# slackhq/nebula

Measured on AMD Instinct MI355X. Metric: GiB/s device-resident AES-256-GCM seal+open, 1300 B pkts, 64 Ki batch, higher is better.
Workload: dtype u8; 1 GPU; C2 AES-256-GCM, 1 tunnel key, 65536 x 1300 B packets, device-resident; packets_per_gpu=65536, payload_bytes_per_pkt=1300, keys=1, cipher=AES-256-GCM, parallelism=1 GPU(s), independent packet shards, no collective

## Files before the change

### nebula_amd/csrc/aes_gcm.hip

```cpp
#include <hip/hip_runtime.h>

#include <atomic>
#include <hip/hip_ext.h>

#include <cstdlib>
#include <cstring>
#include <stdint.h>

#include <type_traits>

#include "../../include/nebula_aead.h"
#include "device_common.hpp"
#include "knobs.hpp"
#include "layout.hpp"
#include "rxwin.hpp"
#include "sched.hpp"
#include "timing.hpp"

#ifdef NEB_ISA_MARKS
#define NEB_MARK(x) asm volatile(";NEBMARK " #x)
#else
#define NEB_MARK(x) ((void)0)
#endif

namespace neb {


struct T0Table {
    uint32_t t[256];
};
constexpr uint8_t kSbox[256] = {
    0x63,0x7c,0x77,0x7b,0xf2,0x6b,0x6f,0xc5,0x30,0x01,0x67,0x2b,0xfe,0xd7,0xab,0x76,
    0xca,0x82,0xc9,0x7d,0xfa,0x59,0x47,0xf0,0xad,0xd4,0xa2,0xaf,0x9c,0xa4,0x72,0xc0,
    0xb7,0xfd,0x93,0x26,0x36,0x3f,0xf7,0xcc,0x34,0xa5,0xe5,0xf1,0x71,0xd8,0x31,0x15,
    0x04,0xc7,0x23,0xc3,0x18,0x96,0x05,0x9a,0x07,0x12,0x80,0xe2,0xeb,0x27,0xb2,0x75,
    0x09,0x83,0x2c,0x1a,0x1b,0x6e,0x5a,0xa0,0x52,0x3b,0xd6,0xb3,0x29,0xe3,0x2f,0x84,
    0x53,0xd1,0x00,0xed,0x20,0xfc,0xb1,0x5b,0x6a,0xcb,0xbe,0x39,0x4a,0x4c,0x58,0xcf,
    0xd0,0xef,0xaa,0xfb,0x43,0x4d,0x33,0x85,0x45,0xf9,0x02,0x7f,0x50,0x3c,0x9f,0xa8,
    0x51,0xa3,0x40,0x8f,0x92,0x9d,0x38,0xf5,0xbc,0xb6,0xda,0x21,0x10,0xff,0xf3,0xd2,
    0xcd,0x0c,0x13,0xec,0x5f,0x97,0x44,0x17,0xc4,0xa7,0x7e,0x3d,0x64,0x5d,0x19,0x73,
    0x60,0x81,0x4f,0xdc,0x22,0x2a,0x90,0x88,0x46,0xee,0xb8,0x14,0xde,0x5e,0x0b,0xdb,
    0xe0,0x32,0x3a,0x0a,0x49,0x06,0x24,0x5c,0xc2,0xd3,0xac,0x62,0x91,0x95,0xe4,0x79,
    0xe7,0xc8,0x37,0x6d,0x8d,0xd5,0x4e,0xa9,0x6c,0x56,0xf4,0xea,0x65,0x7a,0xae,0x08,
    0xba,0x78,0x25,0x2e,0x1c,0xa6,0xb4,0xc6,0xe8,0xdd,0x74,0x1f,0x4b,0xbd,0x8b,0x8a,
    0x70,0x3e,0xb5,0x66,0x48,0x03,0xf6,0x0e,0x61,0x35,0x57,0xb9,0x86,0xc1,0x1d,0x9e,
    0xe1,0xf8,0x98,0x11,0x69,0xd9,0x8e,0x94,0x9b,0x1e,0x87,0xe9,0xce,0x55,0x28,0xdf,
    0x8c,0xa1,0x89,0x0d,0xbf,0xe6,0x42,0x68,0x41,0x99,0x2d,0x0f,0xb0,0x54,0xbb,0x16};

constexpr uint8_t xt(uint8_t a) { return (uint8_t)((a << 1) ^ ((a & 0x80) ? 0x1b : 0)); }
constexpr T0Table make_t0() {
    T0Table r{};
    for (int i = 0; i < 256; i++) {
        uint32_t s = kSbox[i], s2 = xt(kSbox[i]), s3 = s2 ^ s;
        r.t[i] = s2 | (s << 8) | (s << 16) | (s3 << 24);
    }
    return r;
}
__constant__ T0Table c_T0 = make_t0();


__device__ __forceinline__ uint32_t x3(uint32_t a, uint32_t b, uint32_t c) {
    uint32_t r;
    asm("v_bitop3_b32 %0, %1, %2, %3 bitop3:0x96" : "=v"(r) : "v"(a), "v"(b), "v"(c));
    return r;
}
__device__ __forceinline__ uint32_t x3s(uint32_t a, uint32_t b, uint32_t k) {
    uint32_t r;
    asm("v_bitop3_b32 %0, %1, %2, %3 bitop3:0x96" : "=v"(r) : "v"(a), "v"(b), "s"(k));
    return r;
}
__device__ __forceinline__ uint32_t rotl8(uint32_t x) { return __builtin_amdgcn_alignbit(x, x, 24); }
__device__ __forceinline__ uint4 xor4(uint4 a, uint4 b) { return make_uint4(a.x ^ b.x, a.y ^ b.y, a.z ^ b.z, a.w ^ b.w); }
__device__ __forceinline__ uint4 x34(uint4 a, uint4 b, uint4 c) {
    return make_uint4(x3(a.x, b.x, c.x), x3(a.y, b.y, c.y), x3(a.z, b.z, c.z), x3(a.w, b.w, c.w));
}
__device__ __forceinline__ uint4 sel4(bool c, uint4 a, uint4 b) {
    return make_uint4(c ? a.x : b.x, c ? a.y : b.y, c ? a.z : b.z, c ? a.w : b.w);
}
__device__ __forceinline__ uint4 bswap4(uint4 v) { return make_uint4(bswap32(v.x), bswap32(v.y), bswap32(v.z), bswap32(v.w)); }
__device__ __forceinline__ uint4 shfl_xor4(uint4 v, int m) {
    return make_uint4(__shfl_xor(v.x, m), __shfl_xor(v.y, m), __shfl_xor(v.z, m), __shfl_xor(v.w, m));
}
__device__ __forceinline__ uint32_t byte_of(uint32_t w, int k) {
    return k == 0 ? (w & 0xFFu) : (k == 3 ? (w >> 24) : __builtin_amdgcn_ubfe(w, 8 * k, 8));
}

template <class T>
__device__ __forceinline__ T lds_at(const void* base, uint32_t byte_off) {
    return *reinterpret_cast<const T*>(
        __builtin_assume_aligned(reinterpret_cast<const char*>(base) + byte_off, sizeof(T)));
}

__device__ __forceinline__ uint2 lds_b64(const void* base, uint32_t byte_off) {
    typedef uint32_t v2u __attribute__((ext_vector_type(2)));
    typedef const volatile __attribute__((address_space(3))) v2u* lds_ptr;
    const v2u v = *(lds_ptr)__builtin_assume_aligned(reinterpret_cast<const char*>(base) + byte_off, 8);
    return make_uint2(v.x, v.y);
}

__device__ __forceinline__ uint2 ttab_lane_base(uint32_t lane, uint32_t high = 0u) {
    const uint32_t c = lane & 31u, hi = c >> 4;
    return make_uint2((c << 3) | (hi << 2) | high, (c << 3) | ((hi ^ 1u) << 2) | high);
}
__device__ __forceinline__ uint2 ttab_entry(uint32_t i) {
    const uint32_t t = c_T0.t[i >> 5], t2 = __builtin_amdgcn_alignbit(t, t, 16);
    return (i & 16u) ? make_uint2(t2, t) : make_uint2(t, t2);
}

#ifndef NEB_PRIO
#define NEB_PRIO 3
#endif
#ifndef NEB_PRIO_AGE
#define NEB_PRIO_AGE 1
#endif

struct RkRegs {
    const uint32_t* k;
    static constexpr bool kUniform = true;
    static constexpr int kPrioHi = NEB_PRIO, kPrioLo = 0;
    __device__ __forceinline__ uint4 get(int r) const {
        return make_uint4(k[4 * r], k[4 * r + 1], k[4 * r + 2], k[4 * r + 3]);
    }
};
template <int HI, int LO>
struct RkRegsPrio : RkRegs {
    static constexpr int kPrioHi = HI, kPrioLo = LO;
};
struct RkLds {
    const uint4* base;
    static constexpr bool kUniform = false;
    static constexpr int kPrioHi = NEB_PRIO, kPrioLo = 0;
    __device__ __forceinline__ uint4 get(int r) const { return base[r]; }
};

struct TLook {
    const uint2* ttab;
    uint2 lb;
    __device__ __forceinline__ uint32_t t0(uint32_t s, int k) const {
        return lds_at<uint32_t>(ttab, perm(s, lb.x, 0x0C020000u | ((4u + (uint32_t)k) << 8)));
    }
    __device__ __forceinline__ uint32_t t2(uint32_t s, int k) const {
        return lds_at<uint32_t>(ttab, perm(s, lb.y, 0x0C020000u | ((4u + (uint32_t)k) << 8)));
    }
    __device__ __forceinline__ uint32_t t1(uint32_t s, int k) const { return rotl8(t0(s, k)); }
    __device__ __forceinline__ uint32_t t3(uint32_t s, int k) const { return rotl8(t2(s, k)); }
    __device__ __forceinline__ uint32_t t1r(uint32_t s, int k) const { return t0(s, k); }
    __device__ __forceinline__ uint32_t t3r(uint32_t s, int k) const { return t2(s, k); }
    static constexpr bool kFour = false;
};

__device__ __forceinline__ uint32_t ttab4_lane_base(uint32_t lane) {
    const uint32_t c = lane & 31u, hi = c >> 4;
    return ((c << 3) | (hi << 2)) | (1u << 16) | (((c << 3) | ((hi ^ 1u) << 2)) << 24);
}
__device__ __forceinline__ uint2 ttab4_entry(uint32_t i) {
    uint32_t t = c_T0.t[(i >> 5) & 255u];
    if (i & 8192u) t = __builtin_amdgcn_alignbit(t, t, 16);
    const uint32_t t1 = rotl8(t);
    return (i & 16u) ? make_uint2(t1, t) : make_uint2(t, t1);
}
template <uint32_t N, uint32_t THREADS, class F>
__device__ __forceinline__ void fill_ttab(uint2* dst, uint32_t tid, F entry) {
    constexpr uint32_t K = (N + THREADS - 1) / THREADS;
    constexpr bool kWhole = N % THREADS == 0;
    uint2 v[K];
#pragma unroll
    for (uint32_t j = 0; j < K; j++) v[j] = entry((tid + j * THREADS) % N);
#pragma unroll
    for (uint32_t j = 0; j < K; j++)
        if (kWhole || tid + j * THREADS < N) dst[tid + j * THREADS] = v[j];
}
struct TLook4 {
    const uint2* ttab;
    uint32_t lb;
    __device__ __forceinline__ uint32_t at(uint32_t s, int k, uint32_t sel) const {
        return lds_at<uint32_t>(ttab, perm(s, lb, sel | ((4u + (uint32_t)k) << 8)));
    }
    __device__ __forceinline__ uint32_t t0(uint32_t s, int k) const { return at(s, k, 0x0C0C0000u); }
    __device__ __forceinline__ uint32_t t1(uint32_t s, int k) const { return at(s, k, 0x0C0C0003u); }
    __device__ __forceinline__ uint32_t t2(uint32_t s, int k) const { return at(s, k, 0x0C020000u); }
    __device__ __forceinline__ uint32_t t3(uint32_t s, int k) const { return at(s, k, 0x0C020003u); }
    __device__ __forceinline__ uint32_t t1r(uint32_t s, int k) const { return t1(s, k); }
    __device__ __forceinline__ uint32_t t3r(uint32_t s, int k) const { return t3(s, k); }
    static constexpr bool kFour = true;
};

template <int FIRST, class TL, class RK>
__device__ __forceinline__ uint4 aes256_rounds(uint32_t s0, uint32_t s1, uint32_t s2, uint32_t s3, const TL& T,
                                               const RK& rk) {
    uint4 k;
#pragma unroll
    for (int r = FIRST; r < 14; r++) {
        k = rk.get(r);
#if NEB_PRIO
        __builtin_amdgcn_sched_barrier(0);
        __builtin_amdgcn_s_setprio(RK::kPrioHi);
#endif
        const uint32_t a0 = T.t0(s0, 0), a1 = T.t1r(s1, 1), a2 = T.t2(s2, 2), a3 = T.t3r(s3, 3);
        const uint32_t b0 = T.t0(s1, 0), b1 = T.t1r(s2, 1), b2 = T.t2(s3, 2), b3 = T.t3r(s0, 3);
        const uint32_t c0 = T.t0(s2, 0), c1 = T.t1r(s3, 1), c2 = T.t2(s0, 2), c3 = T.t3r(s1, 3);
        const uint32_t d0 = T.t0(s3, 0), d1 = T.t1r(s0, 1), d2 = T.t2(s1, 2), d3 = T.t3r(s2, 3);
#if NEB_PRIO
        __builtin_amdgcn_sched_barrier(0);
        __builtin_amdgcn_s_setprio(RK::kPrioLo);
#endif
        if constexpr (TL::kFour) {
            if constexpr (RK::kUniform) {
                s0 = x3s(x3(a0, a1, a2), a3, k.x);
                s1 = x3s(x3(b0, b1, b2), b3, k.y);
                s2 = x3s(x3(c0, c1, c2), c3, k.z);
                s3 = x3s(x3(d0, d1, d2), d3, k.w);
            } else {
                s0 = x3(x3(a0, a1, a2), a3, k.x);
                s1 = x3(x3(b0, b1, b2), b3, k.y);
                s2 = x3(x3(c0, c1, c2), c3, k.z);
                s3 = x3(x3(d0, d1, d2), d3, k.w);
            }
        } else if constexpr (RK::kUniform) {
            s0 = x3s(a0, a2, k.x) ^ rotl8(a1 ^ a3);
            s1 = x3s(b0, b2, k.y) ^ rotl8(b1 ^ b3);
            s2 = x3s(c0, c2, k.z) ^ rotl8(c1 ^ c3);
            s3 = x3s(d0, d2, k.w) ^ rotl8(d1 ^ d3);
        } else {
            s0 = x3(a0, a2, k.x) ^ rotl8(a1 ^ a3);
            s1 = x3(b0, b2, k.y) ^ rotl8(b1 ^ b3);
            s2 = x3(c0, c2, k.z) ^ rotl8(c1 ^ c3);
            s3 = x3(d0, d2, k.w) ^ rotl8(d1 ^ d3);
        }
    }
    k = rk.get(14);
#if NEB_PRIO
    __builtin_amdgcn_sched_barrier(0);
    __builtin_amdgcn_s_setprio(RK::kPrioHi);
#endif
    const uint32_t a0 = T.t0(s0, 0), a1 = T.t0(s1, 1), a2 = T.t0(s2, 2), a3 = T.t0(s3, 3);
    const uint32_t b0 = T.t0(s1, 0), b1 = T.t0(s2, 1), b2 = T.t0(s3, 2), b3 = T.t0(s0, 3);
    const uint32_t c0 = T.t0(s2, 0), c1 = T.t0(s3, 1), c2 = T.t0(s0, 2), c3 = T.t0(s1, 3);
    const uint32_t d0 = T.t0(s3, 0), d1 = T.t0(s0, 1), d2 = T.t0(s1, 2), d3 = T.t0(s2, 3);
#if NEB_PRIO
    __builtin_amdgcn_sched_barrier(0);
    __builtin_amdgcn_s_setprio(RK::kPrioLo);
#endif
    uint4 o;
    if constexpr (RK::kUniform) {
        o.x = x3s(perm(a1, a0, 0x0C0C0501u), perm(a3, a2, 0x05010C0Cu), k.x);
        o.y = x3s(perm(b1, b0, 0x0C0C0501u), perm(b3, b2, 0x05010C0Cu), k.y);
        o.z = x3s(perm(c1, c0, 0x0C0C0501u), perm(c3, c2, 0x05010C0Cu), k.z);
        o.w = x3s(perm(d1, d0, 0x0C0C0501u), perm(d3, d2, 0x05010C0Cu), k.w);
    } else {
        o.x = x3(perm(a1, a0, 0x0C0C0501u), perm(a3, a2, 0x05010C0Cu), k.x);
        o.y = x3(perm(b1, b0, 0x0C0C0501u), perm(b3, b2, 0x05010C0Cu), k.y);
        o.z = x3(perm(c1, c0, 0x0C0C0501u), perm(c3, c2, 0x05010C0Cu), k.z);
        o.w = x3(perm(d1, d0, 0x0C0C0501u), perm(d3, d2, 0x05010C0Cu), k.w);
    }
    return o;
}

template <class TL, class RK>
__device__ __forceinline__ uint4 aes256_block(uint32_t s0, uint32_t s1, uint32_t s2, uint32_t s3, const TL& T,
                                              const RK& rk) {
    const uint4 k = rk.get(0);
    return aes256_rounds<1>(s0 ^ k.x, s1 ^ k.y, s2 ^ k.z, s3 ^ k.w, T, rk);
}

struct CtrConst {
    uint4 K, L;
    uint32_t k0w;
};

template <class TL, class RK>
__device__ __forceinline__ CtrConst aes_ctr_prep(uint32_t c1, uint32_t c2, const TL& T, const RK& rk) {
    const uint4 k0 = rk.get(0), k1 = rk.get(1), k2 = rk.get(2);
    const uint32_t s0 = k0.x, s1 = c1 ^ k0.y, s2 = c2 ^ k0.z, s3 = k0.w;
    CtrConst c;
    c.k0w = k0.w;
    c.K.x = T.t0(s0, 0) ^ rotl8(T.t0(s1, 1)) ^ T.t2(s2, 2) ^ k1.x;
    c.K.y = T.t0(s1, 0) ^ rotl8(T.t0(s2, 1)) ^ rotl8(T.t2(s0, 3)) ^ k1.y;
    c.K.z = T.t0(s2, 0) ^ rotl8(T.t0(s3, 1) ^ T.t2(s1, 3)) ^ T.t2(s0, 2) ^ k1.z;
    c.K.w = T.t0(s3, 0) ^ rotl8(T.t0(s0, 1) ^ T.t2(s2, 3)) ^ T.t2(s1, 2) ^ k1.w;
    c.L.x = T.t2(c.K.z, 2) ^ rotl8(T.t2(c.K.w, 3)) ^ k2.x;
    c.L.y = rotl8(T.t0(c.K.z, 1)) ^ T.t2(c.K.w, 2) ^ k2.y;
    c.L.z = T.t0(c.K.z, 0) ^ rotl8(T.t0(c.K.w, 1)) ^ k2.z;
    c.L.w = T.t0(c.K.w, 0) ^ rotl8(T.t2(c.K.z, 3)) ^ k2.w;
    return c;
}

template <class TL, class RK>
__device__ __forceinline__ uint4 aes256_ctr_block(const CtrConst& c, uint32_t ctr, const TL& T, const RK& rk) {
    const uint32_t s3 = c.k0w ^ bswap32(ctr);
    const uint32_t t0 = c.K.x ^ T.t3(s3, 3);
    const uint32_t t1 = c.K.y ^ T.t2(s3, 2);
    const uint32_t u0 = x3(c.L.x, T.t0(t0, 0), T.t1(t1, 1));
    const uint32_t u1 = x3(c.L.y, T.t0(t1, 0), T.t3(t0, 3));
    const uint32_t u2 = x3(c.L.z, T.t2(t0, 2), T.t3(t1, 3));
    const uint32_t u3 = x3(c.L.w, T.t2(t1, 2), T.t1(t0, 1));
    return aes256_rounds<3>(u0, u1, u2, u3, T, rk);
}

template <class TL, class RK>
__device__ __forceinline__ CtrConst aes_ctr_prep8(uint32_t c1, uint32_t c2, const TL& T, const RK& rk) {
    CtrConst c = aes_ctr_prep(c1, c2, T, rk);
    const uint4 k2 = rk.get(2);
    c.K.y ^= T.t2(c.k0w, 2);
    c.L.x = rotl8(T.t0(c.K.y, 1)) ^ T.t2(c.K.z, 2) ^ rotl8(T.t2(c.K.w, 3)) ^ k2.x;
    c.L.y = T.t0(c.K.y, 0) ^ rotl8(T.t0(c.K.z, 1)) ^ T.t2(c.K.w, 2) ^ k2.y;
    c.L.z = T.t0(c.K.z, 0) ^ rotl8(T.t0(c.K.w, 1) ^ T.t2(c.K.y, 3)) ^ k2.z;
    c.L.w = T.t0(c.K.w, 0) ^ T.t2(c.K.y, 2) ^ rotl8(T.t2(c.K.z, 3)) ^ k2.w;
    return c;
}

template <class TL, class RK>
__device__ __forceinline__ uint4 aes256_ctr8_block(const CtrConst& c, uint32_t ctr, const TL& T, const RK& rk) {
    const uint32_t t0 = c.K.x ^ T.t3(c.k0w ^ (ctr << 24), 3);
    const uint32_t u0 = c.L.x ^ T.t0(t0, 0);
    const uint32_t u1 = c.L.y ^ T.t3(t0, 3);
    const uint32_t u2 = c.L.z ^ T.t2(t0, 2);
    const uint32_t u3 = c.L.w ^ T.t1(t0, 1);
    return aes256_rounds<3>(u0, u1, u2, u3, T, rk);
}


__device__ __forceinline__ uint4 gf_mulx(uint4 v) {
    uint32_t lsb = v.w & 1u;
// ... 567 lines not shown
        constexpr int CM = decltype(cm)::value;
        CtrConst cc{};
        if constexpr (CM == 2) cc = aes_ctr_prep8(c1, c2, T, rk);
        else if constexpr (CM == 1) cc = aes_ctr_prep(c1, c2, T, rk);
        NEB_MARK(ctr_done);
        auto fast_round = [&](const LaneBlock& b) {
            const uint32_t off = 16u * (b.k - 1u);
            return __all(b.is_ct && off + 16u <= d.len && off >= hdr &&
                         ((d.dst_off | (uint32_t)(uintptr_t)args.arena) & 15u) == 0u);
        };
        auto fast_load = [&](const LaneBlock& b) {
            const uint8_t* sp = args.arena + d.src_off + 16u * (b.k - 1u);
            return __all(((uint32_t)(uintptr_t)sp & 3u) == 0u) ? load_u4_a4(sp) : load_shifted16(sp);
        };
        auto io = [&](const LaneBlock& b, uint4 G, uint4 ks, bool fast, uint4 pre) {
            const uint32_t off = 16u * (b.k - 1u);
            if (fast) {
                const uint4 in = pre;
                if constexpr (CS) {
                    if (cs_on) cs_acc += le16_sum(in);
                }
                const uint4 out = xor4(in, ks);
                *reinterpret_cast<uint4*>(args.arena + d.dst_off + off) = out;
                A = xor4(G, bswap4(OPEN ? in : out));
                return;
            }
            const uint4 in = gcm_lane_load(d, b, args.arena, hdr);
            if constexpr (CS) {
                if (cs_on && b.is_ct) {
                    const uint32_t off = 16u * (b.k - 1u);
                    const uint32_t hi = min(16u, d.len - off), lo = hdr > off ? min(hdr - off, 16u) : 0u;
                    if (lo < hi) {
                        const uint4 v = mask_block(in, hi);
                        cs_acc += le16_sum(xor4(v, mask_block(v, lo)));
                    }
                    if (cs_f - off < 16u) {
                        const uint32_t q = cs_f - off;
                        cs_fk = (block_byte(in, q) << 24) | (block_byte(in, q + 1u) << 16) | (block_byte(ks, q) << 8) |
                                block_byte(ks, q + 1u);
                    }
                }
            }
            A = xor4(G, gcm_lane_io<OPEN>(d, b, in, ks, args.arena, ej0));
        };
        auto horner = [&](uint32_t r) -> uint4 { return r == 0 ? make_uint4(0, 0, 0, 0) : gh.horner(A, lg); };
        auto tround = [&](uint32_t r) {
            NEB_MARK(round_begin);
            if (r < sh.R) {
                const LaneBlock b = lane_block(sh, r, l, lg);
                const bool fast = fast_round(b);
                uint4 pre = make_uint4(0, 0, 0, 0);
                if (fast) pre = fast_load(b);
                const uint4 G = horner(r);
                __builtin_amdgcn_sched_barrier(0);
                uint4 ks = make_uint4(0, 0, 0, 0);
                if (__any(b.is_ct || b.is_len)) ks = gcm_lane_ks<CM>(b, c1, c2, cc, T, rk);
                io(b, G, ks, fast, pre);
            }
            NEB_MARK(round_end);
        };
        for (uint32_t r = 0; __any(r < sh.R); r++) tround(r);
    };
#if NEB_ONE_TRACE
    const uint64_t tp0 = __builtin_amdgcn_s_memrealtime();
#endif
    if (__all(sh.m + 1u < 256u)) rounds(std::integral_constant<int, 2>{});
    else if (__all(sh.m + 1u < 65536u)) rounds(std::integral_constant<int, 1>{});
    else rounds(std::integral_constant<int, 0>{});
    if constexpr (CS) {
        for (uint32_t sft = 1; sft < LPP; sft <<= 1) {
            cs_acc += (uint32_t)__shfl_xor((int)cs_acc, (int)sft);
            cs_fk |= (uint32_t)__shfl_xor((int)cs_fk, (int)sft);
        }
    }
#if NEB_ONE_TRACE
    __builtin_amdgcn_s_waitcnt(0);
    const uint64_t tp1 = __builtin_amdgcn_s_memrealtime();
#endif
#ifdef NEB_WAVE_TRACE
    const uint64_t tq2 = phase_now();
    phase_add(1, tq1, tq2);
#endif
    NEB_MARK(rounds_done);
    uint4 V = gh.final(A, lane, lg);
    NEB_MARK(final_done);
#ifdef NEB_WAVE_TRACE
    const uint64_t tq3 = phase_now();
    phase_add(2, tq2, tq3);
#endif
#if NEB_ONE_TRACE
    __builtin_amdgcn_s_waitcnt(0);
    const uint64_t tp2 = __builtin_amdgcn_s_memrealtime();
    if (lane == 0) printf("  rounds %u  final %u (x10 ns, R=%u)\n", (unsigned)(tp1 - tp0), (unsigned)(tp2 - tp1), sh.R);
#endif
    if constexpr (CS) {
        if (run && cs_on && l == LPP - 1u) V = xor4(V, gcm_csum_fix(d, sh.n, sh.na, cs_acc, cs_fk, args.arena, cs_pow));
    }
    if (run && gcm_finish<OPEN>(d, V, ej0.get(), lane, l, LPP, args.arena)) st = NEB_STATUS_AUTH_FAILED;
    if (valid && l == LPP - 1u) args.status[p] = (int32_t)st;
    NEB_MARK(grp_end);
#ifdef NEB_WAVE_TRACE
    phase_add(3, tq3, phase_now());
#endif
}

__device__ __forceinline__ void load_round_keys(const uint32_t* rec, uint32_t rks[60]) {
#pragma unroll
    for (int i = 0; i < 60; i++) rks[i] = __builtin_amdgcn_readfirstlane(rec[kRecRoundKeys + i]);
}

#ifdef NEB_WAVE_TRACE
constexpr uint32_t kWaveTraceSlots = 64, kWaveTraceWaves = 8192, kWaveTraceCap = kWaveTraceSlots * kWaveTraceWaves;
__device__ uint4 g_wtrace[kWaveTraceCap];
__device__ __forceinline__ void wave_trace(uint32_t lane, uint32_t slot, uint32_t a, uint32_t b, uint64_t t0,
                                           uint64_t t1) {
    const uint32_t w = blockIdx.x * (blockDim.x >> 6) + (threadIdx.x >> 6);
    if (lane == 0u && w < kWaveTraceWaves && slot < kWaveTraceSlots)
        g_wtrace[w * kWaveTraceSlots + slot] = make_uint4(a | 0x80000000u, b, (uint32_t)t0, (uint32_t)t1);
}
#endif


constexpr int kSingleWaves = 16;
constexpr int kSingleWpe = 4;
constexpr int kSingleThreads = kSingleWaves * kWave;

struct SingleLds {
#if NEB_GHASH5
    uint2 full[2 * kWin5 * 32];
#else
    uint4 full[32 * 16];
#endif
    uint4 pos1[8 * 16];
    uint2 ttab[2 * 256 * 32];
    uint4 pos23[2][8 * 16];
#if NEB_GHASH5
    uint4 pos4[8 * 16];
#endif
};
struct SingleLdsCs : SingleLds {
    uint4 pow2[10 * 16];
};

template <bool OPEN, bool CS = false, bool RX = false>
__global__ __launch_bounds__(kSingleThreads, kSingleWpe) void gcm_single_kernel(GcmArgs args) {
    __shared__ std::conditional_t<CS, SingleLdsCs, SingleLds> lds;
    const uint32_t tid = threadIdx.x;
    const uint32_t lane = tid & 63u;
    const uint32_t wave = tid >> 6;
    const uint32_t* srec = args.keys + (size_t)args.key_hint * kKeyRecDwords;
#ifdef NEB_WAVE_TRACE
    const uint64_t tk0 = __builtin_amdgcn_s_memrealtime();
#endif
    uint4 r_full = make_uint4(0, 0, 0, 0), r_h = make_uint4(0, 0, 0, 0), r_p = make_uint4(0, 0, 0, 0);
#if NEB_GHASH5
    static_assert(kSingleThreads >= kWin5 * 32, "one window-table entry per thread");
    const uint32_t f5_p = tid >> 5, f5_v = tid & 31u;
    if (tid < (uint32_t)kWin5 * 32u) {
#pragma unroll
        for (uint32_t j = 0; j < 5u; j++) {
            const uint32_t b = 5u * f5_p + j, bc = min(b, 127u);
            const uint4 c = ld_rec4(srec, kRecFull + 4u * ((bc >> 2) * 16u + (8u >> (bc & 3u))));
            const uint32_t m = (b < 128u && ((f5_v >> (4u - j)) & 1u)) ? ~0u : 0u;
            r_full = make_uint4(r_full.x ^ (c.x & m), r_full.y ^ (c.y & m), r_full.z ^ (c.z & m), r_full.w ^ (c.w & m));
        }
    }
    if (tid < 128u) r_h = ld_rec4(srec, kRecPos1 + 4u * tid);
    if (tid < 384u) r_p = ld_rec4(srec, (tid < 128u ? kRecPos2 : tid < 256u ? kRecPos3 : kRecFull) + 4u * (tid & 127u));
#else
    static_assert(kSingleThreads >= 512, "one full-table entry per thread");
    if (tid < 512u) r_full = ld_rec4(srec, kRecFull + 4u * tid);
    if (tid < 128u) r_h = ld_rec4(srec, kRecPos1 + 4u * tid);
    if (tid < 256u) r_p = ld_rec4(srec, (tid < 128u ? kRecPos2 : kRecPos3) + 4u * (tid & 127u));
#endif
    const TLook4 T{lds.ttab, ttab4_lane_base(lane)};
    fill_ttab<2u * 256u * 32u, kSingleThreads>(lds.ttab, tid, ttab4_entry);
#if NEB_GHASH5
    if (tid < (uint32_t)kWin5 * 32u) {
        lds.full[(2u * f5_p) * 32u + f5_v] = make_uint2(r_full.x, r_full.y);
        lds.full[(2u * f5_p + 1u) * 32u + f5_v] = make_uint2(r_full.z, r_full.w);
    }
    if (tid >= 256u && tid < 384u) lds.pos4[tid & 127u] = r_p;
#else
    if (tid < 512u) lds.full[tid] = r_full;
#endif
    if (tid < 128u) lds.pos1[tid] = r_h;
    if (tid < 256u) lds.pos23[tid >> 7][tid & 127u] = r_p;

    const uint4* cs_pow = nullptr;
    if constexpr (CS) {
        if (tid < 160u) lds.pow2[tid] = ld_rec4(srec, rec_shoup_pow2(tid >> 4) + 4u * (tid & 15u));
        cs_pow = lds.pow2;
    }
    uint32_t rks[60];
    load_round_keys(srec, rks);
    __syncthreads();
    const RkRegs rk{rks};
#if NEB_GHASH5
    const uint32_t tab_off[4] = {(uint32_t)offsetof(SingleLds, pos4), (uint32_t)offsetof(SingleLds, pos23[1]),
#else
    const uint32_t tab_off[4] = {(uint32_t)offsetof(SingleLds, full), (uint32_t)offsetof(SingleLds, pos23[1]),
#endif
                                 (uint32_t)offsetof(SingleLds, pos23[0]), (uint32_t)offsetof(SingleLds, pos1)};
    const GhFullPerm gh{lds.full, &lds, final_perm_lanes(lane, tab_off)};

    const bool key_ok = __builtin_amdgcn_readfirstlane(srec[kRecAlg]) == NEB_ALG_AESGCM;
    uint32_t npkt = args.npkt;
    if (args.npkt_dev) npkt = min(npkt, __builtin_amdgcn_readfirstlane(*args.npkt_dev));
    const uint32_t ngroups = (npkt + kPpw - 1u) / kPpw;
    const uint32_t slots = gridDim.x * kSingleWaves;
    uint32_t main_groups = ngroups;
    if (args.tail_slots && ngroups > slots && ngroups % slots)
        main_groups = ngroups / slots * slots;
#ifdef NEB_WAVE_TRACE
    uint32_t trace_k = 1;
    wave_trace(lane, 0, blockIdx.x << 20 | wave << 16, ~0u, tk0, __builtin_amdgcn_s_memrealtime());
#endif
    auto groups = [&](const auto& rkp) {
        for (uint32_t grp = blockIdx.x + wave * gridDim.x; grp < main_groups; grp += slots) {
#ifdef NEB_WAVE_TRACE
            const uint64_t tc0 = __builtin_amdgcn_s_memrealtime();
#endif
            const uint32_t p = grp * kPpw + lane / kLpp;
            gcm_packet_group<OPEN, CS, RX>(args, p, p < npkt, args.key_hint, key_ok, rkp, gh, T, lane, kLg, cs_pow);
#ifdef NEB_WAVE_TRACE
            wave_trace(lane, trace_k++, blockIdx.x << 20 | wave << 16 | 16u << 8 | 2u << 4 | 1u, grp, tc0,
                       __builtin_amdgcn_s_memrealtime());
#endif
        }
    };
#if NEB_PRIO && NEB_PRIO_AGE
    if (__builtin_amdgcn_readfirstlane(wave) >> 3) groups(RkRegsPrio<NEB_PRIO, 1>{rk});
    else groups(rk);
#else
    groups(rk);
#endif
}

constexpr uint32_t kTailLg = 6, kTailPpw = kWave >> kTailLg;
constexpr uint32_t kTailAll = 0xFFFFFFFFu;
constexpr uint32_t kSmallBatch = 6144;
constexpr int kTailWaves = 8;
struct TailLds {
    uint2 ttab[256 * 32];
    uint4 shoup[kTailLg * 16];
    uint4 pos[8 * 16];
    uint4 m16[16 * 16];
    uint4 hi[3 * 16];
};
static_assert(kTailLg == 6, "GhShoup64: 64 lanes per packet");
template <bool OPEN, bool RX = false>
__global__ __launch_bounds__(kTailWaves * kWave) void gcm_single_tail_kernel(GcmArgs args) {
    __shared__ TailLds lds;
    const uint32_t tid = threadIdx.x, lane = tid & 63u, wave = tid >> 6;
    uint32_t npkt = args.npkt;
    if (args.npkt_dev) npkt = min(npkt, __builtin_amdgcn_readfirstlane(*args.npkt_dev));
    const uint32_t ngroups = (npkt + kPpw - 1u) / kPpw, slots = args.tail_slots;
    uint32_t p0 = 0;
    if (slots != kTailAll) {
        if (ngroups <= slots || ngroups % slots == 0u) return;
        p0 = ngroups / slots * slots * kPpw;
    }
    const uint32_t tgroups = (npkt - p0 + kTailPpw - 1u) / kTailPpw;
    if (blockIdx.x * kTailWaves >= tgroups) return;
    const uint32_t* srec = args.keys + (size_t)args.key_hint * kKeyRecDwords;
    fill_ttab<256u * 32u, kTailWaves * kWave>(lds.ttab, tid, ttab_entry);
    if (tid < 16u * kTailLg) {
        const uint32_t j = tid >> 4, v = tid & 15u;
        lds.shoup[tid] = ld_rec4(srec, rec_shoup_pow2(j) + 4u * v);
    }
    if (tid < 128u) lds.pos[tid] = ld_rec4(srec, kRecPos64 + 4u * tid);
    if (tid < 256u) lds.m16[tid] = ld_rec4(srec, kRecShoup + 4u * tid);
    if (tid < 48u) lds.hi[tid] = ld_rec4(srec, (tid < 16u ? kRecShoup + 15u * 64u : tid < 32u ? kRecShoup32 : kRecShoup48) + 4u * (tid & 15u));
    uint32_t rks[60];
    load_round_keys(srec, rks);
    __syncthreads();
    const TLook T{lds.ttab, ttab_lane_base(lane)};
    const GhShoup64 gh{lds.m16, lds.shoup, lds.pos, lds.hi};
    const bool key_ok = __builtin_amdgcn_readfirstlane(srec[kRecAlg]) == NEB_ALG_AESGCM;
    for (uint32_t t = blockIdx.x * kTailWaves + wave; t < tgroups; t += gridDim.x * kTailWaves) {
        const uint32_t p = p0 + kTailPpw * t + (lane >> kTailLg);
        gcm_packet_group<OPEN, false, RX>(args, p, p < npkt, args.key_hint, key_ok, RkRegs{rks}, gh, T, lane, kTailLg);
    }
}

constexpr uint32_t kOneBytes = 2048;

struct OneArgs {
    neb_desc d;
    const uint32_t* keys;
    uint32_t max_keys, key;
    int32_t* status;
    uint32_t pad_[2];
    uint8_t in[kOneBytes];
};
static_assert(offsetof(OneArgs, in) % 16 == 0, "the packet bytes are read as 16-B blocks");
#ifndef NEB_ONE_FILL_WAVES
#define NEB_ONE_FILL_WAVES 4
#endif
constexpr uint32_t kOneFillThreads = NEB_ONE_FILL_WAVES * kWave;
template <bool OPEN>
__global__ __launch_bounds__(kOneFillThreads) void gcm_one_kernel(OneArgs a) {
    __shared__ TailLds lds;
    const uint32_t tid = threadIdx.x, lane = tid & (kWave - 1u);
#if NEB_ONE_TRACE
    const uint64_t ts0 = __builtin_amdgcn_s_memrealtime();
#endif
    uint64_t kb = (uint64_t)(uintptr_t)__builtin_amdgcn_kernarg_segment_ptr();
    asm volatile("" : "+s"(kb));
    const uint8_t* ka = reinterpret_cast<const uint8_t*>(kb);
    const uint32_t key = a.key;
    const uint32_t* srec = a.keys + (size_t)(key < a.max_keys ? key : 0u) * kKeyRecDwords;
    uint4 warm = make_uint4(0, 0, 0, 0);
    if (tid < kOneBytes / 16u) warm = *reinterpret_cast<const uint4*>(ka + offsetof(OneArgs, in) + 16u * tid);
    for (uint32_t j0 = 0; j0 < 256u * 32u; j0 += 16u * kOneFillThreads) {
        uint2 v[16];
#pragma unroll
        for (uint32_t j = 0; j < 16u; j++) v[j] = ttab_entry(j0 + j * kOneFillThreads + tid);
#pragma unroll
        for (uint32_t j = 0; j < 16u; j++) lds.ttab[j0 + j * kOneFillThreads + tid] = v[j];
    }
    for (uint32_t tdx = tid; tdx < 16u * kTailLg; tdx += kOneFillThreads)
        lds.shoup[tdx] = ld_rec4(srec, rec_shoup_pow2(tdx >> 4) + 4u * (tdx & 15u));
    for (uint32_t tdx = tid; tdx < 128u; tdx += kOneFillThreads) lds.pos[tdx] = ld_rec4(srec, kRecPos64 + 4u * tdx);
    for (uint32_t tdx = tid; tdx < 256u; tdx += kOneFillThreads) lds.m16[tdx] = ld_rec4(srec, kRecShoup + 4u * tdx);
    if (tid < 48u)
        lds.hi[tid] = ld_rec4(srec, (tid < 16u ? kRecShoup + 15u * 64u : tid < 32u ? kRecShoup32 : kRecShoup48) + 4u * (tid & 15u));
    asm volatile("" ::"v"(warm.x), "v"(warm.y), "v"(warm.z), "v"(warm.w));
    __syncthreads();
    if (tid >= kWave) return;
#if NEB_ONE_TRACE
    const uint64_t ts1 = __builtin_amdgcn_s_memrealtime();
#endif
    uint32_t rks[60];
    load_round_keys(srec, rks);
    const TLook T{lds.ttab, ttab_lane_base(lane)};
    const GhShoup64 gh{lds.m16, lds.shoup, lds.pos, lds.hi};
    const bool key_ok = key < a.max_keys && __builtin_amdgcn_readfirstlane(srec[kRecAlg]) == NEB_ALG_AESGCM;
    uint8_t* base = const_cast<uint8_t*>(ka + offsetof(OneArgs, in));
    __shared__ int32_t s_status;
    GcmArgs ga{nullptr, 1u, base, a.keys, a.max_keys, key, &s_status, nullptr, 0u, 0u, nullptr};
    neb_desc d = a.d;
    d.dst_off = a.d.dst_off - (uint64_t)(uintptr_t)base;
#if NEB_ONE_TRACE
    const uint64_t ts2 = __builtin_amdgcn_s_memrealtime();
#endif
    gcm_packet_group<OPEN>(ga, 0u, true, key, key_ok, RkRegs{rks}, gh, T, lane, kTailLg, nullptr, &d);
    one_publish_status(a.status, &s_status);
#if NEB_ONE_TRACE
    __builtin_amdgcn_s_waitcnt(0);
    const uint64_t ts3 = __builtin_amdgcn_s_memrealtime();
    if (lane == 0)
        printf("one %d: fill %u  keys %u  packet %u  (x10 ns)\n", (int)OPEN, (unsigned)(ts1 - ts0), (unsigned)(ts2 - ts1),
               (unsigned)(ts3 - ts2));
#endif
}

constexpr int kOneBatchWaves = 4;
constexpr uint32_t kOneBatchMax = 32;
struct OneBatchDescs {
    neb_desc d[kOneBatchMax];
};
constexpr uint32_t kCombSlot = kOneBytes + 64u;
struct OneBatchLds {
    uint2 ttab[256 * 32];
    struct KeyTabs {
        uint4 shoup[kTailLg * 16];
        uint4 pos[8 * 16];
        uint4 m16[16 * 16];
        uint4 hi[3 * 16];
    } k[kOneBatchWaves];
    uint4 data[kOneBatchWaves][kCombSlot / 16u];
// ... 674 lines not shown
```

Baseline: 857.3 GiB/s.

## Hoist all prologue global loads ahead of LDS table fill and vectorize fill

After: 856.0 GiB/s. No clear change (-0.2%).

```diff
diff --git a/nebula_amd/csrc/aes_gcm.hip b/nebula_amd/csrc/aes_gcm.hip
--- a/nebula_amd/csrc/aes_gcm.hip
+++ b/nebula_amd/csrc/aes_gcm.hip
@@ -153,12 +153,6 @@
     const uint32_t c = lane & 31u, hi = c >> 4;
     return ((c << 3) | (hi << 2)) | (1u << 16) | (((c << 3) | ((hi ^ 1u) << 2)) << 24);
 }
-__device__ __forceinline__ uint2 ttab4_entry(uint32_t i) {
-    uint32_t t = c_T0.t[(i >> 5) & 255u];
-    if (i & 8192u) t = __builtin_amdgcn_alignbit(t, t, 16);
-    const uint32_t t1 = rotl8(t);
-    return (i & 16u) ? make_uint2(t1, t) : make_uint2(t, t1);
-}
 template <uint32_t N, uint32_t THREADS, class F>
 __device__ __forceinline__ void fill_ttab(uint2* dst, uint32_t tid, F entry) {
     constexpr uint32_t K = (N + THREADS - 1) / THREADS;
@@ -169,6 +163,18 @@
 #pragma unroll
     for (uint32_t j = 0; j < K; j++)
         if (kWhole || tid + j * THREADS < N) dst[tid + j * THREADS] = v[j];
+}
+__device__ __forceinline__ void fill_ttab4_pairs(uint2* dst, uint32_t tid, const uint32_t tw[4]) {
+    uint4* d4 = reinterpret_cast<uint4*>(dst);
+    const bool swapped = (tid & 8u) != 0u;
+#pragma unroll
+    for (uint32_t j = 0; j < 8u; j++) {
+        uint32_t t = tw[j & 3u];
+        if (j >= 4u) t = __builtin_amdgcn_alignbit(t, t, 16);
+        const uint32_t t1 = rotl8(t);
+        const uint32_t a = swapped ? t1 : t, b = swapped ? t : t1;
+        d4[tid + j * 1024u] = make_uint4(a, b, a, b);
+    }
 }
 struct TLook4 {
     const uint2* ttab;
@@ -1042,49 +1048,70 @@
 #ifdef NEB_WAVE_TRACE
     const uint64_t tk0 = __builtin_amdgcn_s_memrealtime();
 #endif
-    uint4 r_full = make_uint4(0, 0, 0, 0), r_h = make_uint4(0, 0, 0, 0), r_p = make_uint4(0, 0, 0, 0);
+    static_assert(kSingleThreads == 1024, "fill_ttab4_pairs: 1024 threads");
+    uint32_t tw[4];
+#pragma unroll
+    for (uint32_t k = 0; k < 4u; k++) tw[k] = c_T0.t[(tid >> 4) + 64u * k];
+    uint4 r_c[5], r_h, r_p, r_cs = make_uint4(0, 0, 0, 0);
 #if NEB_GHASH5
     static_assert(kSingleThreads >= kWin5 * 32, "one window-table entry per thread");
     const uint32_t f5_p = tid >> 5, f5_v = tid & 31u;
+#pragma unroll
+    for (uint32_t j = 0; j < 5u; j++) {
+        const uint32_t bc = min(5u * f5_p + j, 127u);
+        r_c[j] = ld_rec4(srec, kRecFull + 4u * ((bc >> 2) * 16u + (8u >> (bc & 3u))));
+    }
+    r_p = ld_rec4(srec, (tid < 128u ? kRecPos2 : tid < 256u ? kRecPos3 : kRecFull) + 4u * (tid & 127u));
+#else
+    static_assert(kSingleThreads >= 512, "one full-table entry per thread");
+    r_c[0] = ld_rec4(srec, kRecFull + 4u * (tid & 511u));
+    r_p = ld_rec4(srec, (tid < 128u ? kRecPos2 : kRecPos3) + 4u * (tid & 127u));
+#endif
+    r_h = ld_rec4(srec, kRecPos1 + 4u * (tid & 127u));
+    if constexpr (CS) {
+        const uint32_t t = min(tid, 159u);
+        r_cs = ld_rec4(srec, rec_shoup_pow2(t >> 4) + 4u * (t & 15u));
+    }
+    const uint32_t slots = gridDim.x * kSingleWaves;
+    const uint32_t grp0 = blockIdx.x + wave * gridDim.x;
+    const uint32_t desc_touch = args.desc[min(grp0 * kPpw + lane / kLpp, args.npkt - 1u)].len;
+    uint32_t rks[60];
+    load_round_keys(srec, rks);
+    const uint32_t alg = __builtin_amdgcn_readfirstlane(srec[kRecAlg]);
+    uint32_t npkt_d = args.npkt;
+    if (args.npkt_dev) npkt_d = __builtin_amdgcn_readfirstlane(*args.npkt_dev);
+    __builtin_amdgcn_sched_barrier(0);
+
+    const TLook4 T{lds.ttab, ttab4_lane_base(lane)};
+    fill_ttab4_pairs(lds.ttab, tid, tw);
+    __builtin_amdgcn_sched_barrier(0);
+
+#if NEB_GHASH5
     if (tid < (uint32_t)kWin5 * 32u) {
+        uint4 r_full = make_uint4(0, 0, 0, 0);
 #pragma unroll
         for (uint32_t j = 0; j < 5u; j++) {
-            const uint32_t b = 5u * f5_p + j, bc = min(b, 127u);
-            const uint4 c = ld_rec4(srec, kRecFull + 4u * ((bc >> 2) * 16u + (8u >> (bc & 3u))));
+            const uint32_t b = 5u * f5_p + j;
             const uint32_t m = (b < 128u && ((f5_v >> (4u - j)) & 1u)) ? ~0u : 0u;
+            const uint4 c = r_c[j];
             r_full = make_uint4(r_full.x ^ (c.x & m), r_full.y ^ (c.y & m), r_full.z ^ (c.z & m), r_full.w ^ (c.w & m));
         }
-    }
-    if (tid < 128u) r_h = ld_rec4(srec, kRecPos1 + 4u * tid);
-    if (tid < 384u) r_p = ld_rec4(srec, (tid < 128u ? kRecPos2 : tid < 256u ? kRecPos3 : kRecFull) + 4u * (tid & 127u));
-#else
-    static_assert(kSingleThreads >= 512, "one full-table entry per thread");
-    if (tid < 512u) r_full = ld_rec4(srec, kRecFull + 4u * tid);
-    if (tid < 128u) r_h = ld_rec4(srec, kRecPos1 + 4u * tid);
-    if (tid < 256u) r_p = ld_rec4(srec, (tid < 128u ? kRecPos2 : kRecPos3) + 4u * (tid & 127u));
-#endif
-    const TLook4 T{lds.ttab, ttab4_lane_base(lane)};
-    fill_ttab<2u * 256u * 32u, kSingleThreads>(lds.ttab, tid, ttab4_entry);
-#if NEB_GHASH5
-    if (tid < (uint32_t)kWin5 * 32u) {
         lds.full[(2u * f5_p) * 32u + f5_v] = make_uint2(r_full.x, r_full.y);
         lds.full[(2u * f5_p + 1u) * 32u + f5_v] = make_uint2(r_full.z, r_full.w);
     }
     if (tid >= 256u && tid < 384u) lds.pos4[tid & 127u] = r_p;
 #else
-    if (tid < 512u) lds.full[tid] = r_full;
+    if (tid < 512u) lds.full[tid] = r_c[0];
 #endif
     if (tid < 128u) lds.pos1[tid] = r_h;
     if (tid < 256u) lds.pos23[tid >> 7][tid & 127u] = r_p;
-
     const uint4* cs_pow = nullptr;
     if constexpr (CS) {
-        if (tid < 160u) lds.pow2[tid] = ld_rec4(srec, rec_shoup_pow2(tid >> 4) + 4u * (tid & 15u));
+        if (tid < 160u) lds.pow2[tid] = r_cs;
         cs_pow = lds.pow2;
     }
-    uint32_t rks[60];
-    load_round_keys(srec, rks);
     __syncthreads();
+    asm volatile("" ::"v"(desc_touch));
     const RkRegs rk{rks};
 #if NEB_GHASH5
     const uint32_t tab_off[4] = {(uint32_t)offsetof(SingleLds, pos4), (uint32_t)offsetof(SingleLds, pos23[1]),
@@ -1094,11 +1121,9 @@
                                  (uint32_t)offsetof(SingleLds, pos23[0]), (uint32_t)offsetof(SingleLds, pos1)};
     const GhFullPerm gh{lds.full, &lds, final_perm_lanes(lane, tab_off)};
 
-    const bool key_ok = __builtin_amdgcn_readfirstlane(srec[kRecAlg]) == NEB_ALG_AESGCM;
-    uint32_t npkt = args.npkt;
-    if (args.npkt_dev) npkt = min(npkt, __builtin_amdgcn_readfirstlane(*args.npkt_dev));
+    const bool key_ok = alg == NEB_ALG_AESGCM;
+    const uint32_t npkt = min(args.npkt, npkt_d);
     const uint32_t ngroups = (npkt + kPpw - 1u) / kPpw;
-    const uint32_t slots = gridDim.x * kSingleWaves;
     uint32_t main_groups = ngroups;
     if (args.tail_slots && ngroups > slots && ngroups % slots)
         main_groups = ngroups / slots * slots;
@@ -1107,7 +1132,7 @@
     wave_trace(lane, 0, blockIdx.x << 20 | wave << 16, ~0u, tk0, __builtin_amdgcn_s_memrealtime());
 #endif
     auto groups = [&](const auto& rkp) {
-        for (uint32_t grp = blockIdx.x + wave * gridDim.x; grp < main_groups; grp += slots) {
+        for (uint32_t grp = grp0; grp < main_groups; grp += slots) {
 #ifdef NEB_WAVE_TRACE
             const uint64_t tc0 = __builtin_amdgcn_s_memrealtime();
 #endif
```
